# yeyupiaoling/PPASR

Hardware: AMD Instinct MI355X
Metric: audio-seconds/s (RTF^-1) Conformer-streaming fbank, batch32 per GPU, ctc_greedy (higher is better)
Workload: dtype f32; 1 GPU; configs[1]: Conformer streaming (configs/conformer.yml), fbank-80, 32 x 10 s utterances per GPU, V=4233, ctc_greedy, features resident in HBM -> token ids + scores on device; global_batch=32, frames=1000, decoder=ctc_greedy, parallelism=utterance-dp1, pipelined=False, gemm=f32

## Files before the change

### ppasr_amd/csrc/front_fused.hip

```cpp
#include <utility>

#include "conformer_kernels.h"
#include "launch.h"

namespace ppasr {

namespace {
constexpr int kGroupRow[5] = {2, 0, 1, 4, 3};
constexpr int kTapCol[5] = {2, 0, 1, 4, 3};
constexpr int kFactor[5] = {2, 0, 1, 3, 1};
constexpr int quad_slab(int t) { return 4 * kFactor[t / 5] + kFactor[t % 5]; }
constexpr int quad_target(int t) {
  const int g = t / 5, k = t % 5;
  if (g == 0) return k == 0 ? 4 : k <= 2 ? 5 : 4;
  const int a = (g == 1 || g == 2) ? 0 : 2;
  return k == 0 ? (a == 0 ? 5 : 4) : k <= 2 ? a : a + 1;
}
constexpr int quad_fold_src(int t) {
  return t == 1 || t == 5 || t == 21 || t == 23 ? 4 : t == 3 || t == 11 || t == 13 ? 5 : -1;
}
constexpr int quad_fold_mask(int t) {
  return t == 1 ? 0xf : t == 3 ? 0x5 : t == 5 ? 0xa : t == 11 ? 0x2 : t == 13 ? 0x1 : t == 21 ? 0x8 : t == 23 ? 0x4 : 0;
}
constexpr bool quad_fold_clear(int t) { return t == 1 || t == 3 || t == 5 || t == 13 || t == 23; }
static_assert(quad_target(0) == 4 && quad_target(2) == 5 && quad_target(10) == 5 && quad_target(12) == 0 &&
                  quad_target(14) == 1 && quad_target(20) == 4 && quad_target(22) == 2 && quad_target(24) == 3,
              "chunk targets");

template <typename Fn, int... I>
__device__ __forceinline__ void static_for(std::integer_sequence<int, I...>, Fn&& fn) {
  (fn(std::integral_constant<int, I>{}), ...);
}

__host__ __device__ inline int quad_xs_stride(int F, int Q) { return F > 8 * Q + 3 ? F : 8 * Q + 3; }
}

template <bool FROM_Y1>
__device__ __forceinline__ void conv2_quad_body(const float* __restrict__ src, const FrontW& fw, float* __restrict__ out,
                                                int T, int F, int Tp, int F2, int M, int m0, const PadSkip& ps,
                                                const int* __restrict__ tile_tab) {
  constexpr int BP = 32, KC = 128, LD = KC + 4, G = KC / 8, NL = 2, N_CHUNKS = 25;
  constexpr int SLOT = BP * LD;
  const int P = (Tp + 1) >> 1;
  const int Q = (F2 + 1) >> 1;
  int r0 = m0 + blockIdx.x * BP, Mlim = M;
  if (tile_tab) {
    const int t = blockIdx.x, nb = tile_tab[0];
    const int* pre = tile_tab + 1;
    if (t >= pre[nb]) return;
    int lo = 0, hi = nb;
    while (hi - lo > 1) {
      const int mid = (lo + hi) >> 1;
      if (pre[mid] <= t) lo = mid;
      else hi = mid;
    }
    const int S = ps.Tp * ps.unit;
    r0 = lo * S + (t - pre[lo]) * BP;
    Mlim = min(M, (lo + 1) * S);
  } else if (pad_block_skippable(ps, r0, BP, M)) {
    return;
  }
  extern __shared__ __attribute__((aligned(16))) float smem[];
  float* const slot0 = smem;
  float* const slot1 = smem + SLOT;
  f32x4* const y2s = reinterpret_cast<f32x4*>(smem + 2 * SLOT);
  float* const w1s = smem + 2 * SLOT + 5 * NL * 4 * kThreads;
  float* const xs = w1s + 10 * 256;
  const int tid = threadIdx.x, lane = lane_id(), wave = wave_id();
  constexpr int tile_stride = 2 * 16 * G * 64;
  const f32x4* wbase = fw.conv2_wp + (size_t)wave * tile_stride;
  auto seg = [&](int h, int slab) { return wbase + (size_t)(16 * h + slab) * G * 64; };
  BRing<1> ring;
  ring_prime(ring, seg(0, quad_slab(0)), 0);
  const int c4 = tid & 31, rbase = tid >> 5;
  const int bp0 = r0 / Q;
  const int FX = quad_xs_stride(F, Q);
  uint32_t pb = 0;
  int yrow[FROM_Y1 ? NL : 1], yp4[FROM_Y1 ? NL : 1], yq4[FROM_Y1 ? NL : 1];
  if constexpr (!FROM_Y1) {
    for (int idx = tid; idx < 10 * 256; idx += kThreads) w1s[idx] = idx < 9 * 256 ? fw.conv1_w[idx] : fw.conv1_b[idx - 9 * 256];
    const int nbp = (min(r0 + BP, Mlim) - 1) / Q - bp0 + 1;
    for (int idx = tid; idx < nbp * 11 * FX; idx += kThreads) {
      const int fr_row = idx / FX, f = idx - fr_row * FX;
      const int bpl = fr_row / 11, fr = fr_row - 11 * bpl;
      const int bp = bp0 + bpl, b = bp / P, p = bp - b * P;
      const int t = min(8 * p + fr, T - 1);
      xs[idx] = f < F ? (src[((size_t)b * T + t) * F + f] - fw.cmvn_mean[f]) * fw.cmvn_istd[f] : 0.f;
    }
#pragma unroll
    for (int i = 0; i < NL; ++i) {
      const int m = r0 + rbase + 16 * i;
      const int bp = m / Q, q = m - bp * Q;
      const uint32_t v = m < Mlim ? (uint32_t)((bp - bp0) * 11 * FX + 8 * q) : 0xffffu;
      pb |= v << (16 * i);
    }
  } else {
#pragma unroll
    for (int i = 0; i < NL; ++i) {
      const int m = r0 + rbase + 16 * i;
      const int bp = m / Q, q = m - bp * Q, b = bp / P, p = bp - b * P;
      yrow[i] = b * T + 4 * p;
      yp4[i] = 4 * p;
      yq4[i] = m < Mlim ? 4 * q : -1;
    }
  }
  auto pbase = [&](int i) { return (int)((pb >> (16 * i)) & 0xffffu); };
  const int lds_off0 = rbase * LD + 4 * c4;
  float xv[9];
  f32x4 wv[3], bv, ya, yv;
  auto y1_step = [&](int i, int h, int r, int c, int step) {
    const int cc = h * 128 + 4 * c4;
    if constexpr (!FROM_Y1) {
      if (step == 0) {
        const int o = pbase(i);
        const float* p = xs + (o == 0xffff ? 0 : o) + 2 * r * FX + 2 * c;
#pragma unroll
        for (int ii = 0; ii < 3; ++ii)
#pragma unroll
          for (int jj = 0; jj < 3; ++jj) xv[ii * 3 + jj] = p[ii * FX + jj];
        ya = f32x4{0.f, 0.f, 0.f, 0.f};
      } else {
#pragma unroll
        for (int j = 3 * (step - 1); j < 3 * step; ++j)
#pragma unroll
          for (int e = 0; e < 4; ++e) ya[e] = fmaf(wv[j % 3][e], xv[j], ya[e]);
        if (step == 3) {
          ya += bv;
#pragma unroll
          for (int e = 0; e < 4; ++e) ya[e] = pbase(i) != 0xffff ? fmaxf(ya[e], 0.f) : 0.f;
        }
      }
      if (step < 3) {
#pragma unroll
        for (int j = 0; j < 3; ++j) wv[j] = *reinterpret_cast<const f32x4*>(w1s + (3 * step + j) * 256 + cc);
        if (step == 2) bv = *reinterpret_cast<const f32x4*>(w1s + 9 * 256 + cc);
      }
    } else {
      if (step == 0) {
        yv = f32x4{0.f, 0.f, 0.f, 0.f};
        if (yq4[i] >= 0 && yp4[i] + r < T && yq4[i] + c < F)
          yv = *reinterpret_cast<const f32x4*>(src + ((size_t)(yrow[i] + r) * F + yq4[i] + c) * 256 + cc);
      } else if (step == 3) {
        ya = yv;
      }
    }
  };
  auto put = [&](float* buf, int i, const f32x4& v) { *reinterpret_cast<f32x4*>(buf + lds_off0 + i * 16 * LD) = v; };
  auto y2row = [&](int c, int i) -> f32x4& { return y2s[(c * NL + i) * kThreads + tid]; };
  f32x4 z2[NL];
  auto build = [&](auto nc, int g, int h, float* buf) {
    constexpr int n = decltype(nc)::value, grp = n / 5, k = n % 5, r = kGroupRow[grp], c = kTapCol[k];
    const int i = g >> 2, step = g & 3;
    y1_step(i, h, r, c, step);
    if (step != 3) return;
    f32x4 v = ya;
    if constexpr (grp == 0) y2row(c, i) = ya;
    if constexpr (grp == 1 || grp == 3) v = ya - y2row(c, i);
    if constexpr (k == 0) {
      z2[i] = v;
      put(buf, i, v);
    } else if constexpr (k == 1 || k == 3) {
      put(buf, i, v - z2[i]);
    } else {
      put(buf, i, v);
    }
  };
  f32x16 acc[6][1][1];
#pragma unroll
  for (int a = 0; a < 6; ++a) acc_zero(acc[a]);
  auto fold = [&](auto tc, int g) {
    constexpr int t = decltype(tc)::value, fs = quad_fold_src(t), mask = quad_fold_mask(t);
    if constexpr (fs >= 0) {
      const int j = g - 4 * NL;
      int seen = 0;
#pragma unroll
      for (int o = 0; o < 4; ++o) {
        if (!((mask >> o) & 1)) continue;
        if (seen++ == j) {
#pragma unroll
          for (int e = 0; e < 16; ++e) asm volatile("v_add_f32 %0, %0, %1" : "+v"(acc[o][0][0][e]) : "v"(acc[fs][0][0][e]));
        }
      }
      if (quad_fold_clear(t) && j == 4) acc_zero(acc[fs]);
    }
  };
  __syncthreads();
#pragma unroll
  for (int g = 0; g < 4 * NL; ++g) {
    build(std::integral_constant<int, 0>{}, g, 0, slot0);
    __builtin_amdgcn_sched_barrier(0);
  }
  __syncthreads();
  for (int h = 0; h < 2; ++h) {
    asm volatile("" : "+s"(wbase));
    if constexpr (!FROM_Y1) {
      asm volatile("" : "+v"(pb));
    } else {
#pragma unroll
      for (int i = 0; i < NL; ++i) asm volatile("" : "+v"(yrow[i]), "+v"(yp4[i]), "+v"(yq4[i]));
    }
    static_for(std::make_integer_sequence<int, N_CHUNKS>{}, [&](auto tc) {
      constexpr int t = decltype(tc)::value;
      float* const cur = ((t + h) & 1) ? slot1 : slot0;
      float* const nxb = ((t + h) & 1) ? slot0 : slot1;
      const f32x4* nseg = t + 1 < N_CHUNKS ? seg(h, quad_slab(t + 1)) : (h == 0 ? seg(1, quad_slab(0)) : nullptr);
      auto side = [&](int g) {
        if (g < 4 * NL) {
          if constexpr (t + 1 < N_CHUNKS) build(std::integral_constant<int, t + 1>{}, g, h, nxb);
          else if (h == 0) build(std::integral_constant<int, 0>{}, g, 1, nxb);
        } else {
          fold(tc, g);
        }
      };
      rb_gemm<1, 1, G, kPF, decltype(side)>(cur, LD, seg(h, quad_slab(t)), 0, nseg, 0, ring, acc[quad_target(t)], side);
      __syncthreads();
    });
  }
  const int col = wave * 32 + (lane & 31);
  const float b2 = fw.conv2_b[col];
#pragma unroll
  for (int r = 0; r < 16; ++r) {
    const int m = r0 + acc_row(r, lane);
    if (m >= Mlim) continue;
    const int bp = m / Q, q = m - bp * Q, b = bp / P, t0 = 2 * (bp - b * P), f0 = 2 * q;
    float* o = out + ((size_t)(b * Tp + t0) * F2 + f0) * 256 + col;
    const bool f1 = f0 + 1 < F2, t1 = t0 + 1 < Tp;
    o[0] = fmaxf(acc[0][0][0][r] + b2, 0.f);
    if (f1) o[256] = fmaxf(acc[1][0][0][r] + b2, 0.f);
    if (t1) o[(size_t)F2 * 256] = fmaxf(acc[2][0][0][r] + b2, 0.f);
    if (t1 && f1) o[(size_t)F2 * 256 + 256] = fmaxf(acc[3][0][0][r] + b2, 0.f);
  }
}

__global__ __launch_bounds__(kThreads) void k_conv12(const float* __restrict__ feats, FrontW fw, float* __restrict__ out,
                                                     int T, int F, int Tp, int F2, int M, int m0, PadSkip ps,
                                                     const int* __restrict__ tile_tab) {
  conv2_quad_body<false>(feats, fw, out, T, F, Tp, F2, M, m0, ps, tile_tab);
}
__global__ __launch_bounds__(kThreads) void k_conv2_pair(const float* __restrict__ y1, FrontW fw, float* __restrict__ out,
                                                         int T1, int F1, int Tp, int F2, int M, int m0, PadSkip ps,
                                                         const int* __restrict__ tile_tab) {
  conv2_quad_body<true>(y1, fw, out, T1, F1, Tp, F2, M, m0, ps, tile_tab);
}

static int quad_tile_pairs(int Q) { return 31 / Q + 2; }
static size_t quad_lds(bool fused, int F, int F2) {
  const int Q = (F2 + 1) / 2;
  return ((size_t)2 * 32 * 132 + (size_t)5 * 2 * 4 * 512 + (fused ? (size_t)10 * 256 + (size_t)quad_tile_pairs(Q) * 11 * quad_xs_stride(F, Q) : 0)) *
         sizeof(float);
}
bool conv2_quad_supported(const FrontW& fw) { return fw.conv2_wp && fw.conv2_k == 3 && fw.conv2_s == 2; }
bool conv12_supported(const FrontW& fw, int F, int F2) {
  const int Q = (F2 + 1) / 2;
  return conv2_quad_supported(fw) && F2 >= 1 && quad_lds(true, F, F2) <= 160 * 1024 &&
         (size_t)quad_tile_pairs(Q) * 11 * quad_xs_stride(F, Q) < 0xffff;
}

void launch_tile_prefix(const PadSkip& ps, int B, int BM, int* tab, hipStream_t st);

static void launch_quad(bool fused, const float* src, const FrontW& fw, float* y2, int B, int T, int F, int Tp, int F2,
                        hipStream_t st, const PadSkip& ps_frames, int* tile_scratch) {
  const int P = (Tp + 1) / 2, Q = (F2 + 1) / 2;
  PadSkip ps = ps_frames;
  ps.Tp = P;
  ps.mul = 2 * ps_frames.mul;
  ps.slack = (ps_frames.slack + 1) / 2;
  ps.unit = Q;
  const int M = B * P * Q;
  const int* no_tab = nullptr;
#define QUAD(GRID, TAB)                                                                                                  \
  do {                                                                                                                 \
    if (fused)                                                                                                         \
      PPASR_LAUNCH(k_conv12, dim3(GRID), dim3(kThreads), quad_lds(true, F, F2), st, src, fw, y2, T, F, Tp, F2, M, 0, ps, \
                   TAB);                                                                                               \
    else                                                                                                               \
      PPASR_LAUNCH(k_conv2_pair, dim3(GRID), dim3(kThreads), quad_lds(false, F, F2), st, src, fw, y2, T, F, Tp, F2, M, 0, \
                   ps, TAB);                                                                                           \
  } while (0)
  if (ps.lens && tile_scratch) {
    launch_tile_prefix(ps, B, 32, tile_scratch, st);
    QUAD(B * ((P * Q + 31) / 32), (const int*)tile_scratch);
    return;
  }
  QUAD((M + 31) / 32, no_tab);
#undef QUAD
}

void launch_conv12(const float* feats, const FrontW& fw, float* y2, int B, int T, int F, int Tp, int F2, hipStream_t st,
                   const PadSkip& ps_frames, int* tile_scratch) {
  launch_quad(true, feats, fw, y2, B, T, F, Tp, F2, st, ps_frames, tile_scratch);
}
void launch_conv2_quad(const float* y1, const FrontW& fw, float* y2, int B, int T1, int F1, int Tp, int F2, hipStream_t st,
                       const PadSkip& ps_frames, int* tile_scratch) {
  launch_quad(false, y1, fw, y2, B, T1, F1, Tp, F2, st, ps_frames, tile_scratch);
}

hipError_t configure_front_fused_kernels() {
  hipError_t e;
#define SET_LDS(fn)                                                                                              \
  e = hipFuncSetAttribute(reinterpret_cast<const void*>(fn), hipFuncAttributeMaxDynamicSharedMemorySize, 160 * 1024); \
  if (e != hipSuccess) return e;
  SET_LDS(k_conv12);
  SET_LDS(k_conv2_pair);
#undef SET_LDS
  return hipSuccess;
}

}
```

Before: 58410 audio-s/s.

## Restructure fused conv1 im2col: register weights, per-row LDS pointers, specialized stride

```diff
diff --git a/ppasr_amd/csrc/front_fused.hip b/ppasr_amd/csrc/front_fused.hip
--- a/ppasr_amd/csrc/front_fused.hip
+++ b/ppasr_amd/csrc/front_fused.hip
@@ -32,10 +32,11 @@
   (fn(std::integral_constant<int, I>{}), ...);
 }
 
-__host__ __device__ inline int quad_xs_stride(int F, int Q) { return F > 8 * Q + 3 ? F : 8 * Q + 3; }
-}
-
-template <bool FROM_Y1>
+__host__ __device__ constexpr int quad_xs_stride(int F, int Q) { return F > 8 * Q + 3 ? F : 8 * Q + 3; }
+constexpr int kFx80 = quad_xs_stride(80, 10);
+}
+
+template <bool FROM_Y1, int FXC = 0>
 __device__ __forceinline__ void conv2_quad_body(const float* __restrict__ src, const FrontW& fw, float* __restrict__ out,
                                                 int T, int F, int Tp, int F2, int M, int m0, const PadSkip& ps,
                                                 const int* __restrict__ tile_tab) {
@@ -74,8 +75,9 @@
   ring_prime(ring, seg(0, quad_slab(0)), 0);
   const int c4 = tid & 31, rbase = tid >> 5;
   const int bp0 = r0 / Q;
-  const int FX = quad_xs_stride(F, Q);
-  uint32_t pb = 0;
+  using lds_cf = const __attribute__((address_space(3))) float;
+  const int FX = FXC ? FXC : quad_xs_stride(F, Q);
+  uint32_t xa[FROM_Y1 ? 1 : NL];
   int yrow[FROM_Y1 ? NL : 1], yp4[FROM_Y1 ? NL : 1], yq4[FROM_Y1 ? NL : 1];
   if constexpr (!FROM_Y1) {
     for (int idx = tid; idx < 10 * 256; idx += kThreads) w1s[idx] = idx < 9 * 256 ? fw.conv1_w[idx] : fw.conv1_b[idx - 9 * 256];
@@ -91,8 +93,7 @@
     for (int i = 0; i < NL; ++i) {
       const int m = r0 + rbase + 16 * i;
       const int bp = m / Q, q = m - bp * Q;
-      const uint32_t v = m < Mlim ? (uint32_t)((bp - bp0) * 11 * FX + 8 * q) : 0xffffu;
-      pb |= v << (16 * i);
+      xa[i] = (uint32_t)(uintptr_t)(lds_cf*)(xs + (m < Mlim ? (bp - bp0) * 11 * FX + 8 * q : 0));
     }
   } else {
 #pragma unroll
@@ -104,58 +105,60 @@
       yq4[i] = m < Mlim ? 4 * q : -1;
     }
   }
-  auto pbase = [&](int i) { return (int)((pb >> (16 * i)) & 0xffffu); };
   const int lds_off0 = rbase * LD + 4 * c4;
-  float xv[9];
-  f32x4 wv[3], bv, ya, yv;
-  auto y1_step = [&](int i, int h, int r, int c, int step) {
+  float xv[NL][3];
+  f32x4 wv[3], bv, ya[NL], yv[NL];
+  constexpr bool W1_REG = !FROM_Y1;
+  f32x4 wreg[10];
+  auto y1_step = [&](int i, int h, int r, int c, int step, auto in_reg) {
+    constexpr bool WR = decltype(in_reg)::value;
     const int cc = h * 128 + 4 * c4;
     if constexpr (!FROM_Y1) {
       if (step == 0) {
-        const int o = pbase(i);
-        const float* p = xs + (o == 0xffff ? 0 : o) + 2 * r * FX + 2 * c;
-#pragma unroll
-        for (int ii = 0; ii < 3; ++ii)
-#pragma unroll
-          for (int jj = 0; jj < 3; ++jj) xv[ii * 3 + jj] = p[ii * FX + jj];
-        ya = f32x4{0.f, 0.f, 0.f, 0.f};
+        ya[i] = f32x4{0.f, 0.f, 0.f, 0.f};
       } else {
 #pragma unroll
-        for (int j = 3 * (step - 1); j < 3 * step; ++j)
-#pragma unroll
-          for (int e = 0; e < 4; ++e) ya[e] = fmaf(wv[j % 3][e], xv[j], ya[e]);
+        for (int j = 0; j < 3; ++j)
+#pragma unroll
+          for (int e = 0; e < 4; ++e) ya[i][e] = fmaf(WR ? wreg[3 * (step - 1) + j][e] : wv[j][e], xv[i][j], ya[i][e]);
         if (step == 3) {
-          ya += bv;
-#pragma unroll
-          for (int e = 0; e < 4; ++e) ya[e] = pbase(i) != 0xffff ? fmaxf(ya[e], 0.f) : 0.f;
+          ya[i] += WR ? wreg[9] : bv;
+#pragma unroll
+          for (int e = 0; e < 4; ++e) ya[i][e] = fmaxf(ya[i][e], 0.f);
         }
+        if (step < 3) asm volatile("" : "+v"(ya[i][0]), "+v"(ya[i][1]), "+v"(ya[i][2]), "+v"(ya[i][3]));
       }
       if (step < 3) {
-#pragma unroll
-        for (int j = 0; j < 3; ++j) wv[j] = *reinterpret_cast<const f32x4*>(w1s + (3 * step + j) * 256 + cc);
-        if (step == 2) bv = *reinterpret_cast<const f32x4*>(w1s + 9 * 256 + cc);
+        lds_cf* p = reinterpret_cast<lds_cf*>((uintptr_t)(xa[i] + 4u * (uint32_t)((2 * r + step) * FX + 2 * c)));
+#pragma unroll
+        for (int jj = 0; jj < 3; ++jj) xv[i][jj] = p[jj];
+        if (!WR && i == (step == 0 ? 0 : NL - 1)) {
+#pragma unroll
+          for (int j = 0; j < 3; ++j) wv[j] = *reinterpret_cast<const f32x4*>(w1s + (3 * step + j) * 256 + cc);
+          if (step == 2) bv = *reinterpret_cast<const f32x4*>(w1s + 9 * 256 + cc);
+        }
       }
     } else {
       if (step == 0) {
-        yv = f32x4{0.f, 0.f, 0.f, 0.f};
+        yv[i] = f32x4{0.f, 0.f, 0.f, 0.f};
         if (yq4[i] >= 0 && yp4[i] + r < T && yq4[i] + c < F)
-          yv = *reinterpret_cast<const f32x4*>(src + ((size_t)(yrow[i] + r) * F + yq4[i] + c) * 256 + cc);
+          yv[i] = *reinterpret_cast<const f32x4*>(src + ((size_t)(yrow[i] + r) * F + yq4[i] + c) * 256 + cc);
       } else if (step == 3) {
-        ya = yv;
+        ya[i] = yv[i];
       }
     }
   };
   auto put = [&](float* buf, int i, const f32x4& v) { *reinterpret_cast<f32x4*>(buf + lds_off0 + i * 16 * LD) = v; };
   auto y2row = [&](int c, int i) -> f32x4& { return y2s[(c * NL + i) * kThreads + tid]; };
   f32x4 z2[NL];
-  auto build = [&](auto nc, int g, int h, float* buf) {
+  auto build = [&](auto nc, int g, int h, float* buf, auto in_reg) {
     constexpr int n = decltype(nc)::value, grp = n / 5, k = n % 5, r = kGroupRow[grp], c = kTapCol[k];
-    const int i = g >> 2, step = g & 3;
-    y1_step(i, h, r, c, step);
+    const int i = g % NL, step = g / NL;
+    y1_step(i, h, r, c, step, in_reg);
     if (step != 3) return;
-    f32x4 v = ya;
-    if constexpr (grp == 0) y2row(c, i) = ya;
-    if constexpr (grp == 1 || grp == 3) v = ya - y2row(c, i);
+    f32x4 v = ya[i];
+    if constexpr (grp == 0) y2row(c, i) = ya[i];
+    if constexpr (grp == 1 || grp == 3) v = ya[i] - y2row(c, i);
     if constexpr (k == 0) {
       z2[i] = v;
       put(buf, i, v);
@@ -187,14 +190,19 @@
   __syncthreads();
 #pragma unroll
   for (int g = 0; g < 4 * NL; ++g) {
-    build(std::integral_constant<int, 0>{}, g, 0, slot0);
+    build(std::integral_constant<int, 0>{}, g, 0, slot0, std::false_type{});
     __builtin_amdgcn_sched_barrier(0);
   }
   __syncthreads();
   for (int h = 0; h < 2; ++h) {
     asm volatile("" : "+s"(wbase));
     if constexpr (!FROM_Y1) {
-      asm volatile("" : "+v"(pb));
+#pragma unroll
+      for (int i = 0; i < NL; ++i) asm volatile("" : "+v"(xa[i]));
+      if constexpr (W1_REG) {
+#pragma unroll
+        for (int j = 0; j < 10; ++j) wreg[j] = *reinterpret_cast<const f32x4*>(w1s + j * 256 + h * 128 + 4 * c4);
+      }
     } else {
 #pragma unroll
       for (int i = 0; i < NL; ++i) asm volatile("" : "+v"(yrow[i]), "+v"(yp4[i]), "+v"(yq4[i]));
@@ -206,8 +214,8 @@
       const f32x4* nseg = t + 1 < N_CHUNKS ? seg(h, quad_slab(t + 1)) : (h == 0 ? seg(1, quad_slab(0)) : nullptr);
       auto side = [&](int g) {
         if (g < 4 * NL) {
-          if constexpr (t + 1 < N_CHUNKS) build(std::integral_constant<int, t + 1>{}, g, h, nxb);
-          else if (h == 0) build(std::integral_constant<int, 0>{}, g, 1, nxb);
+          if constexpr (t + 1 < N_CHUNKS) build(std::integral_constant<int, t + 1>{}, g, h, nxb, std::bool_constant<W1_REG>{});
+          else if (h == 0) build(std::integral_constant<int, 0>{}, g, 1, nxb, std::false_type{});
         } else {
           fold(tc, g);
         }
@@ -232,10 +240,11 @@
   }
 }
 
+template <int FXC>
 __global__ __launch_bounds__(kThreads) void k_conv12(const float* __restrict__ feats, FrontW fw, float* __restrict__ out,
                                                      int T, int F, int Tp, int F2, int M, int m0, PadSkip ps,
                                                      const int* __restrict__ tile_tab) {
-  conv2_quad_body<false>(feats, fw, out, T, F, Tp, F2, M, m0, ps, tile_tab);
+  conv2_quad_body<false, FXC>(feats, fw, out, T, F, Tp, F2, M, m0, ps, tile_tab);
 }
 __global__ __launch_bounds__(kThreads) void k_conv2_pair(const float* __restrict__ y1, FrontW fw, float* __restrict__ out,
                                                          int T1, int F1, int Tp, int F2, int M, int m0, PadSkip ps,
@@ -251,9 +260,7 @@
 }
 bool conv2_quad_supported(const FrontW& fw) { return fw.conv2_wp && fw.conv2_k == 3 && fw.conv2_s == 2; }
 bool conv12_supported(const FrontW& fw, int F, int F2) {
-  const int Q = (F2 + 1) / 2;
-  return conv2_quad_supported(fw) && F2 >= 1 && quad_lds(true, F, F2) <= 160 * 1024 &&
-         (size_t)quad_tile_pairs(Q) * 11 * quad_xs_stride(F, Q) < 0xffff;
+  return conv2_quad_supported(fw) && F2 >= 1 && quad_lds(true, F, F2) <= 160 * 1024;
 }
 
 void launch_tile_prefix(const PadSkip& ps, int B, int BM, int* tab, hipStream_t st);
@@ -270,9 +277,12 @@
   const int* no_tab = nullptr;
 #define QUAD(GRID, TAB)                                                                                                  \
   do {                                                                                                                 \
-    if (fused)                                                                                                         \
-      PPASR_LAUNCH(k_conv12, dim3(GRID), dim3(kThreads), quad_lds(true, F, F2), st, src, fw, y2, T, F, Tp, F2, M, 0, ps, \
-                   TAB);                                                                                               \
+    if (fused && quad_xs_stride(F, Q) == kFx80)                                                                        \
+      PPASR_LAUNCH(k_conv12<kFx80>, dim3(GRID), dim3(kThreads), quad_lds(true, F, F2), st, src, fw, y2, T, F, Tp, F2, M, \
+                   0, ps, TAB);                                                                                        \
+    else if (fused)                                                                                                    \
+      PPASR_LAUNCH(k_conv12<0>, dim3(GRID), dim3(kThreads), quad_lds(true, F, F2), st, src, fw, y2, T, F, Tp, F2, M, 0, \
+                   ps, TAB);                                                                                           \
     else                                                                                                               \
       PPASR_LAUNCH(k_conv2_pair, dim3(GRID), dim3(kThreads), quad_lds(false, F, F2), st, src, fw, y2, T, F, Tp, F2, M, 0, \
                    ps, TAB);                                                                                           \
@@ -300,7 +310,8 @@
 #define SET_LDS(fn)                                                                                              \
   e = hipFuncSetAttribute(reinterpret_cast<const void*>(fn), hipFuncAttributeMaxDynamicSharedMemorySize, 160 * 1024); \
   if (e != hipSuccess) return e;
-  SET_LDS(k_conv12);
+  SET_LDS(k_conv12<kFx80>);
+  SET_LDS(k_conv12<0>);
   SET_LDS(k_conv2_pair);
 #undef SET_LDS
   return hipSuccess;
```

After: 58720 audio-s/s (median of 6 runs). Within noise of the previous version (+0.5%).
